# lhaippp/DMHomo

Hardware: AMD Instinct MI355X
Metric: sampled images/sec (128x128, s_step=32) (higher is better)
Workload: dtype f32; 1 GPU; DGM CFG-Unet dim=64 128x128 bs=25/GPU s_step=32 cond_scale=3 (BASELINE configs[1]); global_batch=25, cfg_mode=streams, hip_graph=True, weights=seeded random init

## Files before the change

dmhomo_amd/_lib.py:

```python
import contextlib
import ctypes as C
import gc
import os

import torch

_HERE = os.path.dirname(os.path.abspath(__file__))
LIB_PATH = os.environ.get('DMH_LIB_PATH') or os.path.join(_HERE, 'libdmhomo_hip.so')

c_f32p = C.c_void_p
c_i64 = C.c_int64
c_int = C.c_int
c_float = C.c_float


ABI_VERSION = 500


class DmhConv(C.Structure):
    _fields_ = [('struct_size', C.c_uint64)] + \
               [(n, C.c_void_p) for n in ('src0', 'src1', 'wpack', 'bias', 'in_coef', 'res', 'res_coef', 'out',
                                          'stats')] + \
               [(n, C.c_int32) for n in ('B', 'Hin', 'Win', 'C0', 'C1', 'Cout', 'KH', 'KW', 'stride', 'upsample2')] + \
               [('in_bound', C.c_void_p), ('in_bound_n', C.c_int32), ('fin_n', C.c_int32), ('fin_w', C.c_void_p),
# ... 11 lines not shown
                ('sqrt_recip_ac', C.c_float), ('sqrt_recipm1_ac', C.c_float), ('sqrt_ac', C.c_float),
                ('sqrt_1m_ac', C.c_float), ('c0', C.c_float), ('c1', C.c_float), ('c2', C.c_float)]


SIGNATURES = {
    'dmh_last_error': (C.c_char_p, []),
    'dmh_version': (c_int, []),
    'dmh_ws_standardize': (c_int, [c_f32p, c_f32p, c_int, c_int, c_float, C.c_void_p]),
    'dmh_conv_pack_floats': (c_i64, [c_int, c_int, c_int, c_int, c_int]),
    'dmh_pack_conv_weight': (c_int, [c_f32p, c_f32p, c_int, c_int, c_int, c_int, c_int, C.c_void_p]),
    'dmh_pack_conv_weights_multi': (c_int, [C.c_void_p, c_int, c_float, C.c_void_p]),
    'dmh_conv_up2_pack_floats': (c_i64, [c_int, c_int]),
    'dmh_pack_conv_weight_up2': (c_int, [c_f32p, c_f32p, c_int, c_int, C.c_void_p]),
    'dmh_conv_tiles': (c_int, [c_int, c_int, c_int, c_int]),
    'dmh_conv2d': (c_int, [C.POINTER(DmhConv), C.c_void_p]),
    'dmh_rows_from_keep': (c_int, [C.c_void_p, c_int, c_int, C.c_void_p, C.c_void_p]),
    'dmh_gn_finalize': (c_int, [c_f32p, c_int, c_f32p, c_f32p, c_f32p, c_i64, c_f32p, c_int, c_int, c_int, c_int,
                                c_float, C.c_void_p, C.c_void_p]),
    'dmh_gn_finalize_bound': (c_int, [c_f32p, c_int, c_f32p, c_f32p, c_f32p, c_i64, c_f32p, c_f32p, c_int, c_int, c_int,
                                      c_int, c_float, C.c_void_p, C.c_void_p]),
    'dmh_gn_silu_residual': (c_int, [c_f32p, c_f32p, c_f32p, c_f32p, c_int, c_int, c_int, C.c_void_p, C.c_void_p]),
    'dmh_gn_silu_residual_stats': (c_int, [c_f32p, c_f32p, c_f32p, c_f32p, c_f32p, c_int, c_int, c_int, c_float, C.c_void_p,
                                           C.c_void_p]),
    'dmh_chan_layernorm': (c_int, [c_f32p, c_f32p, c_f32p, c_f32p, c_i64, c_int, c_float, C.c_void_p, c_i64, C.c_void_p]),
    'dmh_linattn_splits': (c_int, [c_int]),
    'dmh_linattn_partial_floats': (c_i64, [c_int, c_int]),
    'dmh_linattn_context': (c_int, [c_f32p, c_f32p, c_int, c_int, C.c_void_p, C.c_void_p]),
    'dmh_linattn_merge': (c_int, [c_f32p, c_f32p, c_int, c_int, C.c_void_p, C.c_void_p]),
    'dmh_linattn_apply': (c_int, [c_f32p, c_f32p, c_f32p, c_int, c_int, c_float, C.c_void_p, C.c_void_p]),
    'dmh_conv_wgrad_workspace_floats': (c_i64, [c_int, c_int, c_int, c_int, c_int, c_int, c_int]),
# ... 206 lines not shown
```

dmhomo_amd/csrc/conv.hip:

```cpp
#include <stdlib.h>

#include "common.h"

#include "conv_args.h"
#include "weight_image.h"

template <int KH, int KW, int S, int UPS, int KC, int TH, int TW>
struct ConvCfg {
  static constexpr int BM = TH * TW;
  static constexpr int MB = BM / 128;
  static constexpr int IN_H = (TH - 1) * S + KH;
  static constexpr int IN_W = (TW - 1) * S + KW;
  static constexpr int IN_PIX = IN_H * IN_W;
  static constexpr int KCP = KC + 4;
  static constexpr int C4 = KC / 4;
  static constexpr int NLOAD = (IN_PIX * C4 + 255) / 256;
  static constexpr int WL = 64 * C4 / 256;
  static constexpr int PAD = (S == 1) ? (KH / 2) : (KH == 4 ? 1 : 0);
  static constexpr int IN_FLOATS = IN_PIX * KCP;
  static constexpr int W_FLOATS = 64 * KCP;
  static constexpr int EPI_BYTES = 4 * 32 * 68 * 4;
  static constexpr int MAIN_BYTES = (IN_FLOATS + 2 * W_FLOATS) * 4;
  static constexpr int LDS_BYTES = MAIN_BYTES > EPI_BYTES ? MAIN_BYTES : EPI_BYTES;
};
// ... 305 lines not shown
    DMH_REQUIRE(j.src && j.wpack && j.Cout > 0 && j.C0 > 0 && j.C1 >= 0 && (j.KH == 1 || j.KH == 3) &&
                    (j.transposed == 0 || (j.transposed == 1 && j.C1 == 0)),
                "dmh_pack_conv_weights_multi: job %d: stride-1 1x1 / 3x3 weights only (Cout %d, C0 %d, C1 %d, KH %d, transposed %d)",
                i, j.Cout, j.C0, j.C1, j.KH, j.transposed);
  }
  return dmh_f16x3_pack_multi(jobs, njobs, ws_eps, (hipStream_t)stream);
}

extern "C" int dmh_ws_standardize(const float* w, float* w_out, int Cout, int K, float eps, void* stream) {
  DMH_REQUIRE(w && w_out && Cout > 0 && K > 0, "dmh_ws_standardize: bad arguments");
  hipLaunchKernelGGL(ws_standardize_kernel, dim3(Cout), dim3(256), 0, (hipStream_t)stream, w, w_out, K, eps);
  DMH_CHECK_LAUNCH("dmh_ws_standardize");
  return DMH_OK;
}

extern "C" int dmh_conv2d(const DmhConv* d, void* stream) {
  DMH_REQUIRE(d && d->struct_size == sizeof(DmhConv),
              "dmh_conv2d: DmhConv.struct_size is %llu, this library's DmhConv has %llu bytes (header / library mismatch)",
              d ? (unsigned long long)d->struct_size : 0ull, (unsigned long long)sizeof(DmhConv));
  DMH_REQUIRE(d->src0 && d->wpack, "dmh_conv2d: null pointer");
  DMH_REQUIRE(d->B > 0 && d->Hin > 0 && d->Win > 0 && d->C0 > 0 && d->Cout > 0, "dmh_conv2d: bad shape");
  DMH_REQUIRE(d->C0 % 4 == 0 && (!d->src1 || d->C1 % 4 == 0),
              "dmh_conv2d: input channels must be a multiple of 4 (got %d, %d)", d->C0, d->C1);
  DMH_REQUIRE(!(d->in_coef && d->src1), "dmh_conv2d: the GroupNorm prologue applies to a single source");
  DMH_REQUIRE(!(d->res_coef && !d->res), "dmh_conv2d: res_coef without res");
  DMH_REQUIRE(d->Cout % 4 == 0, "dmh_conv2d: Cout must be a multiple of 4 (got %d)", d->Cout);
  DMH_REQUIRE(!d->in_bound || (d->in_coef && d->in_bound_n > 0 && d->in_bound_n <= 64),
              "dmh_conv2d: in_bound needs in_coef and 1..64 bounds per sample (got %d)", d->in_bound_n);
  hipStream_t st = (hipStream_t)stream;
  const int Hout = conv_out_dim(d->Hin, d->KH, d->stride, d->upsample2);
  const int Wout = conv_out_dim(d->Win, d->KW, d->stride, d->upsample2);
  const int key = d->KH * 100 + d->stride * 10 + d->upsample2;
  DMH_REQUIRE(d->KH == d->KW, "dmh_conv2d: non-square kernel");
  if (d->fin_w) {
    DMH_REQUIRE(d->fin_out && d->fin_n > 0 && d->fin_n <= 8, "dmh_conv2d: fin_w needs fin_out and 1 <= fin_n <= 8 (got %d)",
                d->fin_n);
    DMH_REQUIRE(d->KH == 1 && d->stride == 1 && d->Cout <= 64 && use_f16x3(1, 1),
                "dmh_conv2d: the fused final projection rides on the 1x1 fp16-piece kernel with Cout <= 64 (got %dx%d, Cout %d)",
                d->KH, d->KW, d->Cout);
  } else {
    DMH_REQUIRE(d->out, "dmh_conv2d: null pointer");
  }
  DMH_REQUIRE(!d->pix_stats || (d->KH == 1 && d->stride == 1 && d->Cout == 64 && use_f16x3(1, 1)),
              "dmh_conv2d: pix_stats rides on the 1x1 fp16-piece kernel with Cout == 64 (got %dx%d, Cout %d)", d->KH, d->KW,
              d->Cout);
  switch (key) {
    case 110:
      if (use_f16x3(1, 1)) return dmh_f16x3_launch(d, Hout, Wout, st);
      return launch_conv<1, 1, 1, 0, 32, 16, 16>(d, Hout, Wout, st);
    case 310:
      switch (conv3_variant()) {
        case 6: return dmh_wino_launch(d, Hout, Wout, st);
        case 9: return dmh_f16x3_launch(d, Hout, Wout, st);
        default: return launch_conv<3, 3, 1, 0, 32, 16, 16, 2>(d, Hout, Wout, st);
      }
    case 311:
      switch (conv3_variant()) {
        case 6: return dmh_wino_launch(d, Hout, Wout, st);
        case 9: return dmh_f16x3_launch(d, Hout, Wout, st);
        default: return launch_conv<3, 3, 1, 1, 32, 16, 16, 2>(d, Hout, Wout, st);
      }
    case 312:
      DMH_REQUIRE(use_f16x3(3, 1) && !d->src1 && d->Cout % 64 == 0 && !d->stats,
                  "dmh_conv2d: the sub-pixel upsampling conv needs the fp16-piece kernels, one source, Cout %% 64 == 0, no stats");
      return dmh_f16x3_launch_up2(d, Hout, Wout, st);
    case 710:
      if (use_f16x3(7, 1)) return dmh_f16x3_launch(d, Hout, Wout, st);
      return launch_conv<7, 7, 1, 0, 16, 16, 16>(d, Hout, Wout, st);
    case 420:
      if (use_f16x3_s2d(4, 2, d->C0, d->src1 ? d->C1 : 0)) {
        DMH_REQUIRE(!d->in_coef, "dmh_conv2d: the 4x4 / stride-2 conv takes no GroupNorm prologue");
        return dmh_f16x3_launch(d, Hout, Wout, st);
      }
      return launch_conv<4, 4, 2, 0, 16, 8, 16>(d, Hout, Wout, st);
    case 220:
      DMH_REQUIRE(d->Hin % 2 == 0 && d->Win % 2 == 0, "dmh_conv2d: 2x2/s2 needs even input size");
      return launch_conv<2, 2, 2, 0, 16, 8, 16>(d, Hout, Wout, st);
    default:
      dmh_set_error("dmh_conv2d: unsupported variant k=%d stride=%d upsample=%d", d->KH, d->stride, d->upsample2);
      return DMH_EINVAL;
  }
}
```

dmhomo_amd/csrc/conv_args.h:

```cpp
#pragma once
#include "common.h"

typedef float floatx16 __attribute__((ext_vector_type(16)));

struct ConvArgs {
  const float* src0;
  const float* src1;
  const float* wpack;
  const float* bias;
  const float* in_coef;
  const float* res;
  const float* res_coef;
  float* out;
  float* stats;
  const float* oscale;
  const float* in_bound;
  int in_bound_n;
  int fin_n;
  const float* fin_w;
  const float* fin_b;
  float* fin_out;
  float* pix_stats;
  float pix_eps;
  int B, Hin, Win, C0, C1, Cout, Hout, Wout;
// ... 38 lines not shown
  a.tilesY = cdiv(Hout, TH);
  a.ablate = 0;
  a.xcd = 1;
  a.rows = d->rows;
  return a;
}


int64_t dmh_wino_pack_floats(int Cout, int C0, int C1);
int dmh_wino_pack(const float* w, float* wpack, int Cout, int C0, int C1, hipStream_t st);
int dmh_wino_launch(const DmhConv* d, int Hout, int Wout, hipStream_t st);


int64_t dmh_f16x3_pack_floats(int Cout, int C0, int C1, int KH, int KW);
int dmh_f16x3_pack(const float* w, float* wpack, int Cout, int C0, int C1, int KH, int KW, hipStream_t st);
int dmh_f16x3_launch(const DmhConv* d, int Hout, int Wout, hipStream_t st);
int dmh_f16x3_pack_multi(const DmhPackJob* jobs, int njobs, float eps, hipStream_t st);
int64_t dmh_f16x3_up2_pack_floats(int Cout, int C0);
int dmh_f16x3_up2_pack(const float* w, float* wpack, int Cout, int C0, hipStream_t st);
int dmh_f16x3_launch_up2(const DmhConv* d, int Hout, int Wout, hipStream_t st);


struct EpilogueRows {
  static constexpr int EP = 68;
  int b, n0, chn, c4, rsub;
  bool cok;
  float4 bias, ra, rb, s1, s2, osc;

  __device__ __forceinline__ EpilogueRows(const ConvArgs& p, int b_, int n0_) : b(b_), n0(n0_) {
    const int lane = threadIdx.x & 63;
    c4 = lane & 15;
// ... 120 lines not shown
    for (int i = 0; i < NR; ++i) {
      if (okr[i] && (!FIN || p.out)) st4(p.out + oo[i], val[i]);
      const float k = okr[i] ? 1.f : 0.f;
      const float vx = val[i].x * k, vy = val[i].y * k, vz = val[i].z * k, vw = val[i].w * k;
      s1.x += vx;
      s1.y += vy;
      s1.z += vz;
      s1.w += vw;
      s2.x = fmaf(vx, vx, s2.x);
      s2.y = fmaf(vy, vy, s2.y);
      s2.z = fmaf(vz, vz, s2.z);
      s2.w = fmaf(vw, vw, s2.w);
    }
  }

  template <int WM, int WN, int TH>
  __device__ __forceinline__ void write_stats_grid(const ConvArgs& p, float* lds, int ty, int tx, int by = -1) {
    if (by < 0) by = blockIdx.y;
    if (!p.stats) return;
    const int lane = threadIdx.x & 63, wave = threadIdx.x >> 6, tid = threadIdx.x;
    s1.x = rows_sum(s1.x);
    s1.y = rows_sum(s1.y);
    s1.z = rows_sum(s1.z);
    s1.w = rows_sum(s1.w);
    s2.x = rows_sum(s2.x);
    s2.y = rows_sum(s2.y);
    s2.z = rows_sum(s2.z);
    s2.w = rows_sum(s2.w);
    __syncthreads();
    float* red = lds;
    if (lane < 16) {
      float* q = red + (wave * 64 + c4 * 4) * 2;
      q[0] = s1.x;
      q[1] = s2.x;
      q[2] = s1.y;
      q[3] = s2.y;
      q[4] = s1.z;
      q[5] = s2.z;
      q[6] = s1.w;
      q[7] = s2.w;
    }
    __syncthreads();
    if (tid < 128) {
      const int q = tid >> 6, c = tid & 63;
      const int g = WN == 1 ? q : 0, wnq = WN == 1 ? 0 : q;
      const int chan = (by * WN + wnq) * 64 + c;
      const int srow = ty * (TH / 8) + g;
      if (chan < p.Cout && srow * 8 < p.Hout) {
        const int w0 = (g * 2 + 0) * WN + wnq, w1 = (g * 2 + 1) * WN + wnq;
        const float a0 = red[(w0 * 64 + c) * 2 + 0] + red[(w1 * 64 + c) * 2 + 0];
        const float a1 = red[(w0 * 64 + c) * 2 + 1] + red[(w1 * 64 + c) * 2 + 1];
        const int stiles = ((p.Hout + 7) / 8) * p.tilesX;
        float* st = p.stats + ((size_t)(b * stiles + srow * p.tilesX + tx) * p.Cout + chan) * 2;
        st[0] = a0;
        st[1] = a1;
      }
    }
  }

  __device__ __forceinline__ void write_stats(const ConvArgs& p, float* lds, int tile_in_sample) {
    if (!p.stats) return;
// ... 38 lines not shown
```

dmhomo_amd/csrc/conv_f16x3.hip:

```cpp
#include <stdlib.h>

#include "common.h"

#include "conv_args.h"
#include "weight_image.h"

typedef _Float16 half8 __attribute__((ext_vector_type(8)));
typedef _Float16 half4 __attribute__((ext_vector_type(4)));
typedef float float4v __attribute__((ext_vector_type(4)));

namespace {

constexpr int KC = 32;
constexpr int PITCH = 160;
constexpr int STEP_U4 = 4 * 64;

template <int KH, int KW, int S, int UPS, int TH, int TW, int WM, int WN>
struct F16Cfg {
  static_assert(WM * WN == 4, "four waves per workgroup");
  static constexpr bool SUB = UPS == 3;
  static_assert(SUB || TH * TW == WM * 64, "64 pixels per wave");
  static_assert(!SUB || (KH == 2 && KW == 2 && S == 1 && TH == 4 && TW == 16 && WM == 4 && WN == 1), "sub-pixel geometry");
  static constexpr int IN_H = SUB ? TH + 2 : (TH - 1) * S + KH;
  static constexpr int IN_W = SUB ? TW + 2 : (TW - 1) * S + KW;
// ... 4 lines not shown
  static constexpr int ROWP = IN_W * PITCH;
  static constexpr int IN_BYTES = IN_H * ROWP;
  static constexpr int EPI_BYTES = 4 * 32 * EpilogueRows::EP * 4;
  static constexpr int TILE_BYTES = IN_BYTES > EPI_BYTES ? IN_BYTES : EPI_BYTES;
  static constexpr int LDS_BYTES = TILE_BYTES + 16;
};

__device__ __forceinline__ unsigned absbits(float x) { return __float_as_uint(x) & 0x7fffffffu; }

__device__ __forceinline__ int64_t f16x3_frag_floats_dev(int Cout, int C0, int C1, int T) {
  return (int64_t)((Cout + 63) / 64) * ((C0 + KC - 1) / KC + (C1 + KC - 1) / KC) * T * 2 * STEP_U4 * 4;
}

}

template <int KH, int KW, int S, int UPS, int TH, int TW, int WM, int WN>
__global__ __launch_bounds__(256, 2) void conv_f16x3_kernel(ConvArgs p) {
  using Cfg = F16Cfg<KH, KW, S, UPS, TH, TW, WM, WN>;
  constexpr bool PK = UPS == 4;
  constexpr int IN_W = Cfg::IN_W, IN_PIX = Cfg::IN_PIX, NLOAD = Cfg::NLOAD, NTAPS = PK ? (KH * KW + 1) / 2 : KH * KW,
                ROWP = Cfg::ROWP;

  extern __shared__ __attribute__((aligned(16))) float lds[];
  unsigned char* in_tile = reinterpret_cast<unsigned char*>(lds);
  unsigned* mxslot = reinterpret_cast<unsigned*>(in_tile + Cfg::TILE_BYTES);

  const int tid = threadIdx.x;
  const int lane = tid & 63;
  const int wave = tid >> 6;
  const int wave_u = __builtin_amdgcn_readfirstlane(wave);
  const int kg = lane >> 4;
  const int l15 = lane & 15;
  const int wm = wave / WN, wn = wave % WN;
// ... 10 lines not shown
    const int total = nb * gridDim.y, lin = t + by * nb;
    const int q = total >> 3, r = total & 7, xcd = lin & 7, local = lin >> 3;
    const int nl = xcd * q + min(xcd, r) + local;
    if (p.xcd == 2) {
      by = nl % (int)gridDim.y;
      t = nl / (int)gridDim.y;
    } else {
      t = nl % nb;
      by = nl / nb;
    }
  }
  const int tx = t % p.tilesX;
  t /= p.tilesX;
  const int ty = t % p.tilesY;
  const int b = dmh_rows_phys(p.rows, t / p.tilesY);
  const int nt = UPS == 3 ? wm * (int)gridDim.y + by : by * WN + wn;
  const int n0 = UPS == 3 ? by * 64 : nt * 64;

  const int oy0 = ty * TH, ox0 = tx * TW;
  const int iy0 = oy0 * S - Cfg::PAD, ix0 = ox0 * S - Cfg::PAD;
  const int Hlim = UPS == 1 ? p.Hin * 2 : (UPS == 2 ? p.Hin / 2 + 1 : p.Hin);
  const int Wlim = UPS == 1 ? p.Win * 2 : (UPS == 2 ? p.Win / 2 + 1 : p.Win);

  if (tid < 2) mxslot[tid] = 0u;
#ifdef DMH_STAMPS
  unsigned long long tk[8] = {0, 0, 0, 0, 0, 0, 0, 0};
  unsigned long long t_prev, t_now;
#define STAMP(i)                                                                 \
  __builtin_amdgcn_sched_barrier(0);                                             \
  asm volatile("s_memtime %0\n\ts_waitcnt lgkmcnt(0)" : "=s"(t_now)::"memory"); \
  __builtin_amdgcn_sched_barrier(0);                                             \
  tk[i] += t_now - t_prev;                                                       \
  t_prev = t_now;
  asm volatile("s_memtime %0\n\ts_waitcnt lgkmcnt(0)" : "=s"(t_prev)::"memory");
  const unsigned long long t_begin = t_prev;
  const unsigned long long rt_begin = __builtin_amdgcn_s_memrealtime();
#else
#define STAMP(i)
#endif

  static_assert(TW == 16, "a 16-row MFMA block is one tile row");
  int arow[4];
#pragma unroll
  for (int mb = 0; mb < 4; ++mb)
    arow[mb] = UPS == 3 ? (mb + (wm >> 1)) * ROWP + (l15 + (wm & 1)) * PITCH + kg * 16
                        : ((wm * 4 + mb) * S) * ROWP + (l15 * S) * PITCH + (PK ? (kg & 1) : kg) * 16;

  float4v acc[4][4];
#pragma unroll
  for (int mb = 0; mb < 4; ++mb)
#pragma unroll
    for (int nb = 0; nb < 4; ++nb) acc[mb][nb] = float4v{0.f, 0.f, 0.f, 0.f};

  const int nchunks = p.nch0 + p.nch1;
  const int nsteps = nchunks * NTAPS * 2;
  const uint4* wbase = reinterpret_cast<const uint4*>(p.wpack) + (size_t)__builtin_amdgcn_readfirstlane(nt) * nsteps * STEP_U4;

  constexpr bool ROWREUSE = KH == 3 && KW == 3 && S == 1 && UPS != 3 && UPS != 2;
  constexpr int NSTEP = NTAPS * 2;
  constexpr int NB = (NSTEP % 3 == 0 && WN != 1) ? 3 : 2;
  uint4 bq[NB][4];
  auto tap_of = [](int pos) constexpr { return ROWREUSE ? (pos % 3) * 3 + pos / 3 : pos; };
  auto load_b = [&](int buf, int ch_, int st_) {
    if (st_ >= NSTEP) {
      st_ -= NSTEP;
      ch_ += 1;
    }
    if (ch_ >= nchunks) ch_ = nchunks - 1;
    const uint4* src = wbase + ((size_t)(ch_ * NTAPS + tap_of(st_ >> 1)) * 2 + (st_ & 1)) * STEP_U4;
#pragma unroll
    for (int i = 0; i < 4; ++i) bq[buf][i] = src[i * 64 + lane];
  };
#pragma unroll
  for (int i = 0; i < NB - 1; ++i) load_b(i, 0, i);

  constexpr int QS = Cfg::QS, NQ = Cfg::NQ;
  const int c4 = tid & (NQ - 1);
  float4 v[NLOAD];
  constexpr bool PACKPW = KH == 3 && KW == 3 && S == 1 && UPS == 0 && WN == 1;
  int poff[NLOAD], wroff[PACKPW ? 1 : NLOAD];
  const int y0c = min(max(iy0, 0), Hlim - 1), x0c = min(max(ix0, 0), Wlim - 1);
  const int pbase = PACKPW ? (b * p.Hin + y0c) * p.Win + x0c : 0;
  unsigned inside = 0;
#pragma unroll
// ... 142 lines not shown
    const int e_old = e_run;
    int e_ch = e_fix;
    if (!stat) {
      const unsigned bmx = mxslot[ch & 1];
      if (tid == 0) mxslot[(ch + 1) & 1] = 0u;
      e_ch = min(max((int)(__builtin_amdgcn_readfirstlane(bmx) >> 23), 16), 254);
    }
    e_run = max(e_run, e_ch);
    const float sc = __uint_as_float((unsigned)(268 - e_run) << 23);
    if (e_run != e_old && ch > 0) {
      const int fe = 127 + e_old - e_run;
      const float f = fe > 0 ? __uint_as_float((unsigned)fe << 23) : 0.f;
#pragma unroll
      for (int mb = 0; mb < 4; ++mb)
#pragma unroll
        for (int nb = 0; nb < 4; ++nb) acc[mb][nb] *= f;
    }
    const bool more = ch + 1 < nchunks;
    if (more) issue_prep(ch + 1);
#ifdef DMH_STAMPS
    if (p.ablate & 1) {
#pragma unroll
      for (int i = 0; i < NLOAD; ++i)
        if (more) issue_one(i);
    } else
#endif
#pragma unroll
    for (int i = 0; i < NLOAD; ++i) {
      if ((i + 1) * 256 <= IN_PIX * NQ || ((tid + i * 256) >> QS) < IN_PIX) {
        const float si = ((msk >> i) & 1u) ? sc : 0.f;
        uint2 h1, h2;
// ... 33 lines not shown
#pragma unroll
        for (int pl = 0; pl < 2; ++pl)
          ar[ROWREUSE ? r % 5 : 0][pl] = *reinterpret_cast<const half8*>(at + arow[0] + r * ROWP + pl * 64);
    };
#ifdef DMH_STAMPS
    if (!(p.ablate & 2))
#endif
    {
#pragma unroll
      for (int st = 0; st < NSTEP; ++st) {
#ifdef DMH_STAMPS
        if (!(p.ablate & 8))
#endif
        load_b((st + NB - 1) % NB, ch, st + NB - 1);
        __builtin_amdgcn_sched_barrier(0);
        const int pos = st >> 1;
#ifdef DMH_STAMPS
        if (!(p.ablate & 16) || st == 0)
#endif
        {
          if (ROWREUSE) {
            if ((st & 1) == 0) read_rows(pos / 3, pos % 3 == 0 ? 0 : 3 + pos % 3, 4 + pos % 3);
          } else if ((st & 1) == 0) {
            read_a(pos);
          }
        }
        auto afrag = [&](int mb, int pl) -> half8 {
          if constexpr (ROWREUSE) return ar[(mb + pos % 3) % 5][pl];
          else return a[mb][pl];
        };
#define DMH_A(mb, pl) afrag(mb, pl)
#pragma unroll
        for (int mb = 0; mb < 4; ++mb)
#pragma unroll
          for (int nb = 0; nb < 2; ++nb) {
            float4v& c = acc[mb][(st & 1) * 2 + nb];
            const half8 g1 = __builtin_bit_cast(half8, bq[st % NB][nb * 2]), g2 = __builtin_bit_cast(half8, bq[st % NB][nb * 2 + 1]);
            const half8 h1 = DMH_A(mb, 0), h2 = DMH_A(mb, 1);
            asm("v_mfma_f32_16x16x32_f16 %0, %1, %4, %0\n\t"
                "v_mfma_f32_16x16x32_f16 %0, %2, %3, %0\n\t"
                "v_mfma_f32_16x16x32_f16 %0, %1, %3, %0"
                : "+v"(c) : "v"(g1), "v"(g2), "v"(h1), "v"(h2));
          }
#undef DMH_A
      }
    }
#pragma unroll
    for (int mb = 0; mb < 4; mb += 2)
      asm volatile("s_nop 15" : "+v"(acc[mb][0]), "+v"(acc[mb][1]), "+v"(acc[mb][2]), "+v"(acc[mb][3]), "+v"(acc[mb + 1][0]),
                   "+v"(acc[mb + 1][1]), "+v"(acc[mb + 1][2]), "+v"(acc[mb + 1][3]));
    __builtin_amdgcn_sched_barrier(0);
    STAMP(4)
  }

#ifdef DMH_STAMPS
  if (!(p.ablate & 4))
#endif
  {
    constexpr int EP = EpilogueRows::EP;
    const float inv_s = __uint_as_float((unsigned)(e_run - 14) << 23);
    float* wl = lds + wave * (32 * EP);
    EpilogueRows er(p, b, n0);
    if (UPS == 3 && p.oscale) er.osc = ld4(p.oscale + nt * 64 + er.c4 * 4);
    er.osc.x *= inv_s;
    er.osc.y *= inv_s;
    er.osc.z *= inv_s;
    er.osc.w *= inv_s;
    __syncthreads();
#pragma unroll
    for (int hb = 0; hb < 2; ++hb) {
#pragma unroll
      for (int m2 = 0; m2 < 2; ++m2)
#pragma unroll
        for (int nb = 0; nb < 4; ++nb)
          *reinterpret_cast<float4v*>(wl + (m2 * 16 + l15) * EP + nb * 16 + kg * 4) = acc[hb * 2 + m2][nb];
      __builtin_amdgcn_fence(__ATOMIC_RELEASE, "wavefront");
      __builtin_amdgcn_wave_barrier();
      __builtin_amdgcn_fence(__ATOMIC_ACQUIRE, "wavefront");
      if (UPS == 3) er.template store_rows<TW>(p, wl, hb * 32, oy0, ox0, 2, wm >> 1, wm & 1);
      else er.template store_rows<TW, (KH == 1 && KW == 1 && WN == 1 && UPS == 0)>(p, wl, wm * 64 + hb * 32, oy0, ox0);
    }
#ifdef DMH_STAMPS
    STAMP(5)
    if (p.stats && lane == 0 && by == 0) {
      const int stiles = ((p.Hout + 7) / 8) * p.tilesX;
      unsigned long long* d = reinterpret_cast<unsigned long long*>(
                                  p.stats + ((size_t)(b * stiles + (ty * (TH / 8)) * p.tilesX + tx) * p.Cout) * 2) + wave * 8;
      for (int i = 0; i < 6; ++i) d[i] = tk[i];
      d[6] = t_now - t_begin;
      d[7] = __builtin_amdgcn_s_memrealtime() - rt_begin;
    }
#else
    er.template write_stats_grid<WM, WN, TH>(p, lds, ty, tx, by);
#endif
  }
}
#undef STAMP

__global__ __launch_bounds__(64) void f16x3_wscale_kernel(const float* __restrict__ w, float* __restrict__ oscale,
                                                           int Cout, int K) {
  const int o = blockIdx.x;
  float m = 0.f;
  if (o < Cout)
    for (int i = threadIdx.x; i < K; i += 64) m = fmaxf(m, fabsf(w[(size_t)o * K + i]));
  const float s = f16x3_row_scale(m);
  if (threadIdx.x == 0) oscale[o] = s;
}

// ... 124 lines not shown
  const bool s2d = KH == 4;
  if (!s2d && !f16x3_pk(C0, C1, KH)) {
    const DmhPackJob job = {w, nullptr, wpack, Cout, C0, C1, KH, 0};
    return dmh_f16x3_pack_multi(&job, 1, 0.f, st);
  }
  const int64_t frag = f16x3_frag_floats(Cout, C0, C1, KH, KW);
  float* oscale = wpack + frag;
  hipLaunchKernelGGL(f16x3_wscale_kernel, dim3(cdiv(Cout, 64) * 64), dim3(64), 0, st, w, oscale, Cout, C0 * KH * KW);
  const int64_t total = frag * 2;
  hipLaunchKernelGGL(pack_f16x3_weight_kernel, dim3((unsigned)cdiv64(total, 256)), dim3(256), 0, st, w, oscale,
                     reinterpret_cast<_Float16*>(wpack), Cout, C0, s2d ? 4 : 25, s2d ? 4 * C0 / KC : 1, total, s2d ? 1 : 0);
  DMH_CHECK_LAUNCH("dmh_pack_conv_weight(f16x3)");
  return DMH_OK;
}

template <int KH, int KW, int S, int UPS, int TH, int TW, int WM, int WN>
static int launch_f16x3(const DmhConv* d, int Hout, int Wout, hipStream_t st) {
  using Cfg = F16Cfg<KH, KW, S, UPS, TH, TW, WM, WN>;
  ConvArgs a = fill_conv_args(d, Hout, Wout, KC, TH, TW);
  if (UPS == 2) a.nch0 = 4 * a.C0 / KC;
  a.oscale = d->wpack + f16x3_frag_floats(d->Cout, a.C0, a.C1, UPS == 2 ? 4 : KH, UPS == 2 ? 4 : KW);
#ifdef DMH_STAMPS
  if (const char* e = getenv("DMH_WINO_ABLATE")) a.ablate = atoi(e);
#endif
  auto kern = conv_f16x3_kernel<KH, KW, S, UPS, TH, TW, WM, WN>;
  DMH_RAISE_LDS_ONCE(kern, Cfg::LDS_BYTES, "dmh_conv2d(f16x3)");
  static const int xcd_deep = [] {
    const char* e = getenv("DMH_CONV_XCD_DEEP");
    return e ? atoi(e) : 32;
  }();
  if (xcd_deep > 0 && Hout <= xcd_deep && cdiv(a.Cout, 64 * WN) > 1) a.xcd = 2;
  dim3 grid(a.tilesX * a.tilesY * a.B, cdiv(a.Cout, 64 * WN));
  hipLaunchKernelGGL(kern, grid, dim3(256), Cfg::LDS_BYTES, st, a);
  DMH_CHECK_LAUNCH("dmh_conv2d(f16x3)");
  return DMH_OK;
}

__global__ void subpixel_weight_kernel(const float* __restrict__ w, float* __restrict__ wv, int Cout, int Cin) {
  const int64_t idx = (int64_t)blockIdx.x * blockDim.x + threadIdx.x;
  const int64_t total = (int64_t)4 * Cout * Cin * 4;
  if (idx >= total) return;
  const int tb = idx & 1, ta = (idx >> 1) & 1;
  int64_t r = idx >> 2;
  const int c = r % Cin;
  r /= Cin;
  const int o = r % Cout, par = r / Cout;
  const int dy = par >> 1, dx = par & 1;
// ... 19 lines not shown

int dmh_f16x3_launch_up2(const DmhConv* d, int Hout, int Wout, hipStream_t st) {
  using Cfg = F16Cfg<2, 2, 1, 3, 4, 16, 4, 1>;
  ConvArgs a = fill_conv_args(d, Hout, Wout, KC, 4, 16);
  a.tilesX = cdiv(d->Win, 16);
  a.tilesY = cdiv(d->Hin, 4);
  a.oscale = d->wpack + f16x3_frag_floats(4 * d->Cout, a.C0, 0, 2, 2);
  auto kern = conv_f16x3_kernel<2, 2, 1, 3, 4, 16, 4, 1>;
  DMH_RAISE_LDS_ONCE(kern, Cfg::LDS_BYTES, "dmh_conv2d(f16x3 sub-pixel)");
  dim3 grid(a.tilesX * a.tilesY * a.B, cdiv(a.Cout, 64));
  hipLaunchKernelGGL(kern, grid, dim3(256), Cfg::LDS_BYTES, st, a);
  DMH_CHECK_LAUNCH("dmh_conv2d(f16x3 sub-pixel)");
  return DMH_OK;
}

int dmh_f16x3_launch(const DmhConv* d, int Hout, int Wout, hipStream_t st) {
  const bool wide = d->Cout % 128 == 0;
  if (d->KH == 4) {
    return wide ? launch_f16x3<2, 2, 1, 2, 8, 16, 2, 2>(d, Hout, Wout, st)
                : launch_f16x3<2, 2, 1, 2, 16, 16, 4, 1>(d, Hout, Wout, st);
  }
  if (d->KH == 7) {
    if (f16x3_pk(d->C0, d->src1 ? d->C1 : 0, 7)) return launch_f16x3<7, 7, 1, 4, 16, 16, 4, 1>(d, Hout, Wout, st);
    return launch_f16x3<7, 7, 1, 0, 16, 16, 4, 1>(d, Hout, Wout, st);
  }
  if (d->KH == 1) {
    return wide ? launch_f16x3<1, 1, 1, 0, 8, 16, 2, 2>(d, Hout, Wout, st)
                : launch_f16x3<1, 1, 1, 0, 16, 16, 4, 1>(d, Hout, Wout, st);
  }
  if (d->upsample2) {
    return wide ? launch_f16x3<3, 3, 1, 1, 8, 16, 2, 2>(d, Hout, Wout, st)
                : launch_f16x3<3, 3, 1, 1, 16, 16, 4, 1>(d, Hout, Wout, st);
  }
  if (wide) return launch_f16x3<3, 3, 1, 0, 8, 16, 2, 2>(d, Hout, Wout, st);
  DMH_REQUIRE(17 * (int64_t)d->Win + 17 < 65536, "dmh_conv2d: 3x3 with Cout %% 128 != 0 supports Win <= 3853 (got %d)", d->Win);
  return launch_f16x3<3, 3, 1, 0, 16, 16, 4, 1>(d, Hout, Wout, st);
}
```

dmhomo_amd/ops.py:

```python
import ctypes as C

import os

import torch

from . import _lib
from ._lib import call, ptr, lib

F32 = torch.float32


def _empty(shape, like, dtype=F32):
    return torch.empty(shape, device=like.device, dtype=dtype)


def ws_standardize(w, eps=1e-5, out=None):
    w = w.detach().contiguous()
    out = torch.empty_like(w) if out is None else out
    cout = w.shape[0]
    call('dmh_ws_standardize', ptr(w), ptr(out), cout, w.numel() // cout, float(eps))
    return out


class PackBatch:
# ... 77 lines not shown
CONV_LOG = None


def rows_from_keep(keep, extra=0):
    B = keep.shape[0]
    rows = torch.empty((1 + B + extra,), device=keep.device, dtype=torch.int32)
    call('dmh_rows_from_keep', ptr(keep, torch.uint8), B, int(extra), ptr(rows, torch.int32))
    return rows


def _rows(rows):
    return ptr(rows, torch.int32)


def conv2d(pc, src0, src1=None, in_coef=None, res=None, res_coef=None, want_stats=False, in_bound=None, final=None,
           keep_out=True, pixel_stats=False, eps=1e-5, fin_out=None, rows=None):
    B, H, W, c0 = src0.shape
    assert c0 == pc.c0 and (pc.c1 == 0) == (src1 is None), (src0.shape, pc.c0, pc.c1)
    if src1 is not None:
        assert src1.shape == (B, H, W, pc.c1), (src1.shape, pc.c1)
    ho, wo = conv_out_hw(pc, H, W)
    assert keep_out or final is not None
    out = _empty((B, ho, wo, pc.cout), src0) if keep_out else None
    fin_w = fin_b = None
    if final is not None:
        fin_w, fin_b = final
        assert fin_w.shape[1] == pc.cout and fin_w.is_contiguous() and not want_stats, (fin_w.shape, pc.cout)
        if fin_out is None:
            fin_out = _empty((B, fin_w.shape[0], ho, wo), src0)
        assert fin_out.shape == (B, fin_w.shape[0], ho, wo) and fin_out.is_contiguous() and fin_out.dtype == F32
    else:
        assert fin_out is None
    pst = None
    if pixel_stats:
        assert final is None and not want_stats and pc.cout == 64 and pc.k == 1, (pc.cout, pc.k)
        pst = _empty((B, ho * wo, 2), src0)
    stats = None
    if want_stats:
        tiles = lib().dmh_conv_tiles(ho, wo, pc.k, pc.stride)
        stats = _empty((B, tiles, pc.cout, 2), src0)
    if res is not None:
        assert res.shape == (B, ho, wo, pc.cout), (res.shape, (B, ho, wo, pc.cout))
    d = _lib.DmhConv(C.sizeof(_lib.DmhConv), ptr(src0), ptr(src1), ptr(pc.wpack), ptr(pc.bias), ptr(in_coef), ptr(res), ptr(res_coef),
                     ptr(out), ptr(stats), B, H, W, pc.c0, pc.c1, pc.cout, pc.k, pc.k, pc.stride, pc.upsample2,
                     ptr(in_bound), 0 if in_bound is None else in_bound.shape[1],
                     0 if fin_w is None else fin_w.shape[0], ptr(fin_w), ptr(fin_b), ptr(fin_out), ptr(pst), float(eps), _rows(rows))
    if CONV_LOG is not None:
        e0, e1 = torch.cuda.Event(enable_timing=True), torch.cuda.Event(enable_timing=True)
        e0.record()
        call('dmh_conv2d', C.byref(d))
        e1.record()
        CONV_LOG.append((e0, e1, pc.k, pc.stride, B, ho, wo, pc.c0 + pc.c1, pc.cout, pc.upsample2, in_coef is not None))
    else:
        call('dmh_conv2d', C.byref(d))
    if final is not None:
        return out, fin_out
    if pixel_stats:
        return out, pst
    return (out, stats) if want_stats else out


def _ss_arg(ss, B, Cc):
    if ss is None:
        return None, 0
    assert ss.stride(1) == 1 and ss.shape[0] == B and ss.shape[1] == 2 * Cc
    return C.c_void_p(ss.data_ptr()), ss.stride(0)


def gn_finalize(stats, gamma, beta, hw, groups, ss=None, eps=1e-5, want_bound=False, rows=None):
# ... 1102 lines not shown
```

include/dmhomo_hip.h:

```cpp
#ifndef DMHOMO_HIP_H
#define DMHOMO_HIP_H

#include <stdint.h>

#ifdef __cplusplus
extern "C" {
#endif

#define DMH_OK 0
#define DMH_EINVAL (-1)
#define DMH_ELAUNCH (-2)

const char* dmh_last_error(void);
#define DMH_ABI_VERSION 500
int dmh_version(void);


int dmh_ws_standardize(const float* w, float* w_out, int Cout, int K, float eps, void* stream);

int64_t dmh_conv_pack_floats(int Cout, int C0, int C1, int KH, int KW);

int dmh_pack_conv_weight(const float* w_oihw, float* wpack, int Cout, int C0, int C1, int KH, int KW,
                         void* stream);
typedef struct DmhPackJob {
// ... 26 lines not shown
  int32_t stride;
  int32_t upsample2;
  const float* in_bound;
  int32_t in_bound_n;
  int32_t fin_n;
  const float* fin_w;
  const float* fin_b;
  float* fin_out;
  float* pix_stats;
  float pix_eps;
  const int32_t* rows;
} DmhConv;

int dmh_conv_tiles(int Hout, int Wout, int KH, int stride);
int dmh_conv2d(const DmhConv* d, void* stream);


int dmh_gn_finalize(const float* stats, int tiles, const float* gamma, const float* beta, const float* ss,
                    int64_t ss_stride, float* coef, int B, int C, int groups, int hw, float eps, const int32_t* rows,
                    void* stream);

int dmh_gn_finalize_bound(const float* stats, int tiles, const float* gamma, const float* beta, const float* ss,
                          int64_t ss_stride, float* coef, float* bound, int B, int C, int groups, int hw, float eps,
                          const int32_t* rows, void* stream);

int dmh_gn_silu_residual(const float* y, const float* coef, const float* res, float* out, int B, int HW, int C,
                         const int32_t* rows, void* stream);

int dmh_gn_silu_residual_stats(const float* y, const float* coef, const float* res, float* out, float* pstats, int B,
                               int HW, int C, float eps, const int32_t* rows, void* stream);
// ... 237 lines not shown
```

Measured before the change: 89.53 images/s.

## Add narrow 32-channel-per-wave conv variant for small-spatial fp16-piece layers

Adds a CW=32 template variant of the fp16-piece conv kernel in which each wave covers 32 output channels instead of 64, doubling the grid's channel dimension. A heuristic picks it by default for small-spatial, wide-channel 3x3 and 4x4-stride-2 layers (few tiles), where the grid would otherwise have too few blocks to fill the GPU. The epilogue and stats writing are adapted to the half-width channel split. It also exposes an explicit layout override entry point. The cost is more blocks that each reload the same input tile and fewer MFMAs per A-fragment read.

```diff
diff --git a/dmhomo_amd/_lib.py b/dmhomo_amd/_lib.py
--- a/dmhomo_amd/_lib.py
+++ b/dmhomo_amd/_lib.py
@@ -49,6 +49,7 @@
     'dmh_pack_conv_weight_up2': (c_int, [c_f32p, c_f32p, c_int, c_int, C.c_void_p]),
     'dmh_conv_tiles': (c_int, [c_int, c_int, c_int, c_int]),
     'dmh_conv2d': (c_int, [C.POINTER(DmhConv), C.c_void_p]),
+    'dmh_conv2d_layout': (c_int, [C.POINTER(DmhConv), c_int, C.c_void_p]),
     'dmh_rows_from_keep': (c_int, [C.c_void_p, c_int, c_int, C.c_void_p, C.c_void_p]),
     'dmh_gn_finalize': (c_int, [c_f32p, c_int, c_f32p, c_f32p, c_f32p, c_i64, c_f32p, c_int, c_int, c_int, c_int,
                                 c_float, C.c_void_p, C.c_void_p]),
diff --git a/dmhomo_amd/csrc/conv.hip b/dmhomo_amd/csrc/conv.hip
--- a/dmhomo_amd/csrc/conv.hip
+++ b/dmhomo_amd/csrc/conv.hip
@@ -343,7 +343,7 @@
   return DMH_OK;
 }
 
-extern "C" int dmh_conv2d(const DmhConv* d, void* stream) {
+static int conv2d_impl(const DmhConv* d, int layout, void* stream) {
   DMH_REQUIRE(d && d->struct_size == sizeof(DmhConv),
               "dmh_conv2d: DmhConv.struct_size is %llu, this library's DmhConv has %llu bytes (header / library mismatch)",
               d ? (unsigned long long)d->struct_size : 0ull, (unsigned long long)sizeof(DmhConv));
@@ -373,20 +373,26 @@
   DMH_REQUIRE(!d->pix_stats || (d->KH == 1 && d->stride == 1 && d->Cout == 64 && use_f16x3(1, 1)),
               "dmh_conv2d: pix_stats rides on the 1x1 fp16-piece kernel with Cout == 64 (got %dx%d, Cout %d)", d->KH, d->KW,
               d->Cout);
+  if (layout != 0) {
+    const bool f16 = key == 420 ? use_f16x3_s2d(4, 2, d->C0, d->src1 ? d->C1 : 0)
+                                : (use_f16x3(d->KH, d->stride) && (key == 110 || key == 310 || key == 311));
+    DMH_REQUIRE(f16, "dmh_conv2d_layout: only the fp16-piece 1x1 / 3x3 / 4x4-stride-2 kernels have layouts to choose from "
+                     "(k=%d stride=%d upsample=%d)", d->KH, d->stride, d->upsample2);
+  }
   switch (key) {
     case 110:
-      if (use_f16x3(1, 1)) return dmh_f16x3_launch(d, Hout, Wout, st);
+      if (use_f16x3(1, 1)) return dmh_f16x3_launch(d, Hout, Wout, st, layout);
       return launch_conv<1, 1, 1, 0, 32, 16, 16>(d, Hout, Wout, st);
     case 310:
       switch (conv3_variant()) {
         case 6: return dmh_wino_launch(d, Hout, Wout, st);
-        case 9: return dmh_f16x3_launch(d, Hout, Wout, st);
+        case 9: return dmh_f16x3_launch(d, Hout, Wout, st, layout);
         default: return launch_conv<3, 3, 1, 0, 32, 16, 16, 2>(d, Hout, Wout, st);
       }
     case 311:
       switch (conv3_variant()) {
         case 6: return dmh_wino_launch(d, Hout, Wout, st);
-        case 9: return dmh_f16x3_launch(d, Hout, Wout, st);
+        case 9: return dmh_f16x3_launch(d, Hout, Wout, st, layout);
         default: return launch_conv<3, 3, 1, 1, 32, 16, 16, 2>(d, Hout, Wout, st);
       }
     case 312:
@@ -394,12 +400,12 @@
                   "dmh_conv2d: the sub-pixel upsampling conv needs the fp16-piece kernels, one source, Cout %% 64 == 0, no stats");
       return dmh_f16x3_launch_up2(d, Hout, Wout, st);
     case 710:
-      if (use_f16x3(7, 1)) return dmh_f16x3_launch(d, Hout, Wout, st);
+      if (use_f16x3(7, 1)) return dmh_f16x3_launch(d, Hout, Wout, st, layout);
       return launch_conv<7, 7, 1, 0, 16, 16, 16>(d, Hout, Wout, st);
     case 420:
       if (use_f16x3_s2d(4, 2, d->C0, d->src1 ? d->C1 : 0)) {
         DMH_REQUIRE(!d->in_coef, "dmh_conv2d: the 4x4 / stride-2 conv takes no GroupNorm prologue");
-        return dmh_f16x3_launch(d, Hout, Wout, st);
+        return dmh_f16x3_launch(d, Hout, Wout, st, layout);
       }
       return launch_conv<4, 4, 2, 0, 16, 8, 16>(d, Hout, Wout, st);
     case 220:
@@ -410,3 +416,11 @@
       return DMH_EINVAL;
   }
 }
+
+extern "C" int dmh_conv2d(const DmhConv* d, void* stream) { return conv2d_impl(d, 0, stream); }
+
+extern "C" int dmh_conv2d_layout(const DmhConv* d, int layout, void* stream) {
+  DMH_REQUIRE(layout >= 0 && layout <= 2, "dmh_conv2d_layout: layout is 0 (the library's choice), 1 (wide) or 2 (narrow), got %d",
+              layout);
+  return conv2d_impl(d, layout, stream);
+}
diff --git a/dmhomo_amd/csrc/conv_args.h b/dmhomo_amd/csrc/conv_args.h
--- a/dmhomo_amd/csrc/conv_args.h
+++ b/dmhomo_amd/csrc/conv_args.h
@@ -76,7 +76,7 @@
 
 int64_t dmh_f16x3_pack_floats(int Cout, int C0, int C1, int KH, int KW);
 int dmh_f16x3_pack(const float* w, float* wpack, int Cout, int C0, int C1, int KH, int KW, hipStream_t st);
-int dmh_f16x3_launch(const DmhConv* d, int Hout, int Wout, hipStream_t st);
+int dmh_f16x3_launch(const DmhConv* d, int Hout, int Wout, hipStream_t st, int layout = 0);
 int dmh_f16x3_pack_multi(const DmhPackJob* jobs, int njobs, float eps, hipStream_t st);
 int64_t dmh_f16x3_up2_pack_floats(int Cout, int C0);
 int dmh_f16x3_up2_pack(const float* w, float* wpack, int Cout, int C0, hipStream_t st);
@@ -227,7 +227,7 @@
     }
   }
 
-  template <int WM, int WN, int TH>
+  template <int WM, int WN, int TH, int CW = 64>
   __device__ __forceinline__ void write_stats_grid(const ConvArgs& p, float* lds, int ty, int tx, int by = -1) {
     if (by < 0) by = blockIdx.y;
     if (!p.stats) return;
@@ -254,10 +254,10 @@
       q[7] = s2.w;
     }
     __syncthreads();
-    if (tid < 128) {
+    if (tid < (CW == 32 ? 64 : 128)) {
       const int q = tid >> 6, c = tid & 63;
-      const int g = WN == 1 ? q : 0, wnq = WN == 1 ? 0 : q;
-      const int chan = (by * WN + wnq) * 64 + c;
+      const int g = WN == 1 ? q : 0, wnq = WN == 1 ? 0 : (CW == 32 ? c >> 5 : q);
+      const int chan = CW == 32 ? by * 64 + c : (by * WN + wnq) * 64 + c;
       const int srow = ty * (TH / 8) + g;
       if (chan < p.Cout && srow * 8 < p.Hout) {
         const int w0 = (g * 2 + 0) * WN + wnq, w1 = (g * 2 + 1) * WN + wnq;
diff --git a/dmhomo_amd/csrc/conv_f16x3.hip b/dmhomo_amd/csrc/conv_f16x3.hip
--- a/dmhomo_amd/csrc/conv_f16x3.hip
+++ b/dmhomo_amd/csrc/conv_f16x3.hip
@@ -42,9 +42,12 @@
 
 }
 
-template <int KH, int KW, int S, int UPS, int TH, int TW, int WM, int WN>
+template <int KH, int KW, int S, int UPS, int TH, int TW, int WM, int WN, int CW = 64>
 __global__ __launch_bounds__(256, 2) void conv_f16x3_kernel(ConvArgs p) {
   using Cfg = F16Cfg<KH, KW, S, UPS, TH, TW, WM, WN>;
+  static_assert(CW == 64 || (CW == 32 && WM == 2 && WN == 2 && UPS != 3 && UPS != 4), "output channels per wave");
+  constexpr int HPW = CW / 32;
+  constexpr int NBK = CW / 16;
   constexpr bool PK = UPS == 4;
   constexpr int IN_W = Cfg::IN_W, IN_PIX = Cfg::IN_PIX, NLOAD = Cfg::NLOAD, NTAPS = PK ? (KH * KW + 1) / 2 : KH * KW,
                 ROWP = Cfg::ROWP;
@@ -85,8 +88,9 @@
   t /= p.tilesX;
   const int ty = t % p.tilesY;
   const int b = dmh_rows_phys(p.rows, t / p.tilesY);
-  const int nt = UPS == 3 ? wm * (int)gridDim.y + by : by * WN + wn;
+  const int nt = UPS == 3 ? wm * (int)gridDim.y + by : (by * WN + wn) * CW / 64;
   const int n0 = UPS == 3 ? by * 64 : nt * 64;
+  const int chalf = CW == 32 ? wn : 0;
 
   const int oy0 = ty * TH, ox0 = tx * TW;
   const int iy0 = oy0 * S - Cfg::PAD, ix0 = ox0 * S - Cfg::PAD;
@@ -117,18 +121,19 @@
     arow[mb] = UPS == 3 ? (mb + (wm >> 1)) * ROWP + (l15 + (wm & 1)) * PITCH + kg * 16
                         : ((wm * 4 + mb) * S) * ROWP + (l15 * S) * PITCH + (PK ? (kg & 1) : kg) * 16;
 
-  float4v acc[4][4];
+  float4v acc[4][NBK];
 #pragma unroll
   for (int mb = 0; mb < 4; ++mb)
 #pragma unroll
-    for (int nb = 0; nb < 4; ++nb) acc[mb][nb] = float4v{0.f, 0.f, 0.f, 0.f};
+    for (int nb = 0; nb < NBK; ++nb) acc[mb][nb] = float4v{0.f, 0.f, 0.f, 0.f};
 
   const int nchunks = p.nch0 + p.nch1;
   const int nsteps = nchunks * NTAPS * 2;
-  const uint4* wbase = reinterpret_cast<const uint4*>(p.wpack) + (size_t)__builtin_amdgcn_readfirstlane(nt) * nsteps * STEP_U4;
+  const uint4* wbase = reinterpret_cast<const uint4*>(p.wpack) + (size_t)__builtin_amdgcn_readfirstlane(nt) * nsteps * STEP_U4 +
+                       __builtin_amdgcn_readfirstlane(chalf) * STEP_U4;
 
   constexpr bool ROWREUSE = KH == 3 && KW == 3 && S == 1 && UPS != 3 && UPS != 2;
-  constexpr int NSTEP = NTAPS * 2;
+  constexpr int NSTEP = NTAPS * HPW;
   constexpr int NB = (NSTEP % 3 == 0 && WN != 1) ? 3 : 2;
   uint4 bq[NB][4];
   auto tap_of = [](int pos) constexpr { return ROWREUSE ? (pos % 3) * 3 + pos / 3 : pos; };
@@ -138,7 +143,7 @@
       ch_ += 1;
     }
     if (ch_ >= nchunks) ch_ = nchunks - 1;
-    const uint4* src = wbase + ((size_t)(ch_ * NTAPS + tap_of(st_ >> 1)) * 2 + (st_ & 1)) * STEP_U4;
+    const uint4* src = wbase + ((size_t)(ch_ * NTAPS + tap_of(st_ / HPW)) * 2 + (st_ % HPW)) * STEP_U4;
 #pragma unroll
     for (int i = 0; i < 4; ++i) bq[buf][i] = src[i * 64 + lane];
   };
@@ -311,7 +316,7 @@
 #pragma unroll
       for (int mb = 0; mb < 4; ++mb)
 #pragma unroll
-        for (int nb = 0; nb < 4; ++nb) acc[mb][nb] *= f;
+        for (int nb = 0; nb < NBK; ++nb) acc[mb][nb] *= f;
     }
     const bool more = ch + 1 < nchunks;
     if (more) issue_prep(ch + 1);
@@ -375,14 +380,14 @@
 #endif
         load_b((st + NB - 1) % NB, ch, st + NB - 1);
         __builtin_amdgcn_sched_barrier(0);
-        const int pos = st >> 1;
+        const int pos = st / HPW;
 #ifdef DMH_STAMPS
         if (!(p.ablate & 16) || st == 0)
 #endif
         {
           if (ROWREUSE) {
-            if ((st & 1) == 0) read_rows(pos / 3, pos % 3 == 0 ? 0 : 3 + pos % 3, 4 + pos % 3);
-          } else if ((st & 1) == 0) {
+            if (st % HPW == 0) read_rows(pos / 3, pos % 3 == 0 ? 0 : 3 + pos % 3, 4 + pos % 3);
+          } else if (st % HPW == 0) {
             read_a(pos);
           }
         }
@@ -395,7 +400,7 @@
         for (int mb = 0; mb < 4; ++mb)
 #pragma unroll
           for (int nb = 0; nb < 2; ++nb) {
-            float4v& c = acc[mb][(st & 1) * 2 + nb];
+            float4v& c = acc[mb][(st % HPW) * 2 + nb];
             const half8 g1 = __builtin_bit_cast(half8, bq[st % NB][nb * 2]), g2 = __builtin_bit_cast(half8, bq[st % NB][nb * 2 + 1]);
             const half8 h1 = DMH_A(mb, 0), h2 = DMH_A(mb, 1);
             asm("v_mfma_f32_16x16x32_f16 %0, %1, %4, %0\n\t"
@@ -407,9 +412,14 @@
       }
     }
 #pragma unroll
-    for (int mb = 0; mb < 4; mb += 2)
-      asm volatile("s_nop 15" : "+v"(acc[mb][0]), "+v"(acc[mb][1]), "+v"(acc[mb][2]), "+v"(acc[mb][3]), "+v"(acc[mb + 1][0]),
-                   "+v"(acc[mb + 1][1]), "+v"(acc[mb + 1][2]), "+v"(acc[mb + 1][3]));
+    for (int mb = 0; mb < 4; mb += 2) {
+      if constexpr (NBK == 4)
+        asm volatile("s_nop 15" : "+v"(acc[mb][0]), "+v"(acc[mb][1]), "+v"(acc[mb][2]), "+v"(acc[mb][3]), "+v"(acc[mb + 1][0]),
+                     "+v"(acc[mb + 1][1]), "+v"(acc[mb + 1][2]), "+v"(acc[mb + 1][3]));
+      else
+        asm volatile("s_nop 15" : "+v"(acc[0][0]), "+v"(acc[0][1]), "+v"(acc[1][0]), "+v"(acc[1][1]), "+v"(acc[2][0]),
+                     "+v"(acc[2][1]), "+v"(acc[3][0]), "+v"(acc[3][1]));
+    }
     __builtin_amdgcn_sched_barrier(0);
     STAMP(4)
   }
@@ -427,18 +437,22 @@
     er.osc.y *= inv_s;
     er.osc.z *= inv_s;
     er.osc.w *= inv_s;
+    if (CW == 32) er.cok = er.cok && (er.c4 >> 3) == chalf;
+    const int cq = CW == 32 ? (er.c4 & 7) * 4 : er.c4 * 4;
     __syncthreads();
 #pragma unroll
     for (int hb = 0; hb < 2; ++hb) {
 #pragma unroll
       for (int m2 = 0; m2 < 2; ++m2)
 #pragma unroll
-        for (int nb = 0; nb < 4; ++nb)
+        for (int nb = 0; nb < NBK; ++nb)
           *reinterpret_cast<float4v*>(wl + (m2 * 16 + l15) * EP + nb * 16 + kg * 4) = acc[hb * 2 + m2][nb];
       __builtin_amdgcn_fence(__ATOMIC_RELEASE, "wavefront");
       __builtin_amdgcn_wave_barrier();
       __builtin_amdgcn_fence(__ATOMIC_ACQUIRE, "wavefront");
-      if (UPS == 3) er.template store_rows<TW>(p, wl, hb * 32, oy0, ox0, 2, wm >> 1, wm & 1);
+      if constexpr (CW == 32)
+        er.template store_rows_fn<TW>(p, [wl, cq](int rr) { return ld4(wl + rr * EP + cq); }, wm * 64 + hb * 32, oy0, ox0);
+      else if (UPS == 3) er.template store_rows<TW>(p, wl, hb * 32, oy0, ox0, 2, wm >> 1, wm & 1);
       else er.template store_rows<TW, (KH == 1 && KW == 1 && WN == 1 && UPS == 0)>(p, wl, wm * 64 + hb * 32, oy0, ox0);
     }
 #ifdef DMH_STAMPS
@@ -452,7 +466,7 @@
       d[7] = __builtin_amdgcn_s_memrealtime() - rt_begin;
     }
 #else
-    er.template write_stats_grid<WM, WN, TH>(p, lds, ty, tx, by);
+    er.template write_stats_grid<WM, WN, TH, CW>(p, lds, ty, tx, by);
 #endif
   }
 }
@@ -607,7 +621,7 @@
   return DMH_OK;
 }
 
-template <int KH, int KW, int S, int UPS, int TH, int TW, int WM, int WN>
+template <int KH, int KW, int S, int UPS, int TH, int TW, int WM, int WN, int CW = 64>
 static int launch_f16x3(const DmhConv* d, int Hout, int Wout, hipStream_t st) {
   using Cfg = F16Cfg<KH, KW, S, UPS, TH, TW, WM, WN>;
   ConvArgs a = fill_conv_args(d, Hout, Wout, KC, TH, TW);
@@ -616,14 +630,14 @@
 #ifdef DMH_STAMPS
   if (const char* e = getenv("DMH_WINO_ABLATE")) a.ablate = atoi(e);
 #endif
-  auto kern = conv_f16x3_kernel<KH, KW, S, UPS, TH, TW, WM, WN>;
+  auto kern = conv_f16x3_kernel<KH, KW, S, UPS, TH, TW, WM, WN, CW>;
   DMH_RAISE_LDS_ONCE(kern, Cfg::LDS_BYTES, "dmh_conv2d(f16x3)");
   static const int xcd_deep = [] {
     const char* e = getenv("DMH_CONV_XCD_DEEP");
     return e ? atoi(e) : 32;
   }();
-  if (xcd_deep > 0 && Hout <= xcd_deep && cdiv(a.Cout, 64 * WN) > 1) a.xcd = 2;
-  dim3 grid(a.tilesX * a.tilesY * a.B, cdiv(a.Cout, 64 * WN));
+  if (xcd_deep > 0 && Hout <= xcd_deep && cdiv(a.Cout, CW * WN) > 1) a.xcd = 2;
+  dim3 grid(a.tilesX * a.tilesY * a.B, cdiv(a.Cout, CW * WN));
   hipLaunchKernelGGL(kern, grid, dim3(256), Cfg::LDS_BYTES, st, a);
   DMH_CHECK_LAUNCH("dmh_conv2d(f16x3)");
   return DMH_OK;
@@ -673,9 +687,23 @@
   return DMH_OK;
 }
 
-int dmh_f16x3_launch(const DmhConv* d, int Hout, int Wout, hipStream_t st) {
+static bool f16x3_has_narrow(const DmhConv* d) {
+  return d->Cout % 128 == 0 && (d->KH == 4 || (d->KH == 3 && d->upsample2 != 2));
+}
+
+static bool f16x3_narrow_rule(const DmhConv* d, int Hout, int Wout) {
+  const int tiles = cdiv(Hout, 8) * cdiv(Wout, 16), Cin = d->C0 + (d->src1 ? d->C1 : 0);
+  return f16x3_has_narrow(d) && tiles <= 2 && tiles * (d->Cout / 128) <= 8 && !(d->KH == 3 && Cin < d->Cout);
+}
+
+int dmh_f16x3_launch(const DmhConv* d, int Hout, int Wout, hipStream_t st, int layout) {
   const bool wide = d->Cout % 128 == 0;
+  const bool narrow = layout == 2 || (layout == 0 && f16x3_narrow_rule(d, Hout, Wout));
+  DMH_REQUIRE(layout == 0 || (layout == 1 && wide && d->KH != 7) || (layout == 2 && f16x3_has_narrow(d)),
+              "dmh_conv2d_layout: layout %d does not exist for this shape (k=%d, upsample=%d, Cout %d)", layout, d->KH,
+              d->upsample2, d->Cout);
   if (d->KH == 4) {
+    if (narrow) return launch_f16x3<2, 2, 1, 2, 8, 16, 2, 2, 32>(d, Hout, Wout, st);
     return wide ? launch_f16x3<2, 2, 1, 2, 8, 16, 2, 2>(d, Hout, Wout, st)
                 : launch_f16x3<2, 2, 1, 2, 16, 16, 4, 1>(d, Hout, Wout, st);
   }
@@ -688,9 +716,11 @@
                 : launch_f16x3<1, 1, 1, 0, 16, 16, 4, 1>(d, Hout, Wout, st);
   }
   if (d->upsample2) {
+    if (narrow) return launch_f16x3<3, 3, 1, 1, 8, 16, 2, 2, 32>(d, Hout, Wout, st);
     return wide ? launch_f16x3<3, 3, 1, 1, 8, 16, 2, 2>(d, Hout, Wout, st)
                 : launch_f16x3<3, 3, 1, 1, 16, 16, 4, 1>(d, Hout, Wout, st);
   }
+  if (narrow) return launch_f16x3<3, 3, 1, 0, 8, 16, 2, 2, 32>(d, Hout, Wout, st);
   if (wide) return launch_f16x3<3, 3, 1, 0, 8, 16, 2, 2>(d, Hout, Wout, st);
   DMH_REQUIRE(17 * (int64_t)d->Win + 17 < 65536, "dmh_conv2d: 3x3 with Cout %% 128 != 0 supports Win <= 3853 (got %d)", d->Win);
   return launch_f16x3<3, 3, 1, 0, 16, 16, 4, 1>(d, Hout, Wout, st);
diff --git a/dmhomo_amd/ops.py b/dmhomo_amd/ops.py
--- a/dmhomo_amd/ops.py
+++ b/dmhomo_amd/ops.py
@@ -115,7 +115,7 @@
 
 
 def conv2d(pc, src0, src1=None, in_coef=None, res=None, res_coef=None, want_stats=False, in_bound=None, final=None,
-           keep_out=True, pixel_stats=False, eps=1e-5, fin_out=None, rows=None):
+           keep_out=True, pixel_stats=False, eps=1e-5, fin_out=None, rows=None, layout=None):
     B, H, W, c0 = src0.shape
     assert c0 == pc.c0 and (pc.c1 == 0) == (src1 is None), (src0.shape, pc.c0, pc.c1)
     if src1 is not None:
@@ -146,14 +146,15 @@
                      ptr(out), ptr(stats), B, H, W, pc.c0, pc.c1, pc.cout, pc.k, pc.k, pc.stride, pc.upsample2,
                      ptr(in_bound), 0 if in_bound is None else in_bound.shape[1],
                      0 if fin_w is None else fin_w.shape[0], ptr(fin_w), ptr(fin_b), ptr(fin_out), ptr(pst), float(eps), _rows(rows))
+    entry = ('dmh_conv2d', C.byref(d)) if layout is None else ('dmh_conv2d_layout', C.byref(d), int(layout))
     if CONV_LOG is not None:
         e0, e1 = torch.cuda.Event(enable_timing=True), torch.cuda.Event(enable_timing=True)
         e0.record()
-        call('dmh_conv2d', C.byref(d))
+        call(*entry)
         e1.record()
         CONV_LOG.append((e0, e1, pc.k, pc.stride, B, ho, wo, pc.c0 + pc.c1, pc.cout, pc.upsample2, in_coef is not None))
     else:
-        call('dmh_conv2d', C.byref(d))
+        call(*entry)
     if final is not None:
         return out, fin_out
     if pixel_stats:
diff --git a/include/dmhomo_hip.h b/include/dmhomo_hip.h
--- a/include/dmhomo_hip.h
+++ b/include/dmhomo_hip.h
@@ -64,6 +64,7 @@
 
 int dmh_conv_tiles(int Hout, int Wout, int KH, int stride);
 int dmh_conv2d(const DmhConv* d, void* stream);
+int dmh_conv2d_layout(const DmhConv* d, int layout, void* stream);
 
 
 int dmh_gn_finalize(const float* stats, int tiles, const float* gamma, const float* beta, const float* ss,
```

Result: faster. 90.58 images/s (median of 6 runs) (+1.2%).
